# NethermindEth/latticefold

Hardware: AMD Instinct MI355X
Metric: folding-prover steps/sec (one NIFSProver::prove per step), GoldilocksRingNTT (higher is better)
Workload: dtype u64; 1 GPU; C4: GoldilocksRingNTT R1CS->CCS, m=N=2^20 rows, wit_len=262144, L=4, B=2^16, b=2, K=16, kappa=26, t=3; parallelism=replicas x1

## Files before the change

### latticefold_amd/csrc/lf_ctx.h

```cpp
#pragma once
#include <hip/hip_runtime.h>
#include <assert.h>
#include <string.h>

#include <atomic>
#include <chrono>
#include <condition_variable>
#include <functional>
#include <future>
#include <thread>
#include <map>
#include <memory>
#include <mutex>
#include <string>
#include <vector>

#include "../../include/lfhip.h"
#include "bb_capi.h"
#include "lf_ctx_core.h"
#include "lf_common.h"
#include "lf_dist.h"
#include "lf_kernels.h"
#include "lf_sb.h"
#include "lf_verify.h"
// ... 243 lines not shown
        if (tr) { tr->t.set_basis(nullptr, nullptr); if (tr->bb) tr->bb->set_basis(nullptr, nullptr); }
    }
    const u64 *ring_in(const u64 *p, size_t elems) {
        if (!p) return p;
        keep.emplace_back(new std::vector<u64>(p, p + elems * RE));
        c->xb.to_int(keep.back()->data(), elems * 8);
        return keep.back()->data();
    }
    const u64 *ext_in(const u64 *p, size_t n) {
        if (!p) return p;
        keep.emplace_back(new std::vector<u64>(p, p + n * TAU));
        c->xb.to_int(keep.back()->data(), n);
        return keep.back()->data();
    }
    void ring_out(u64 *p, size_t elems) { if (p) c->xb.to_ext(p, elems * 8); }
    void ext_out(u64 *p, size_t n) { if (p) c->xb.to_ext(p, n); }
    void transcript(lf_transcript *t) {
        tr = t;
        if (t->bb) t->bb->set_basis(c->xb.T, c->xb.Ti);
        else t->t.set_basis(c->xb.T, c->xb.Ti);
    }
};
#define LF_XB(c) ((c) && (c)->xb.on && !t_xb_active)
int fold_impl(lf_ctx *c, Transcript &tr, SideState *S , u64 *lcccs_out, lf_witness **w_out, u64 *proof);
int commit_download(lf_ctx *c, const u64 *dev, size_t words, u64 *host);
int commit_parts_i8g(lf_ctx *c, const unsigned char *D, size_t ldn, u32 NP, u64 *out_dev);
int sb_cut_parts(lf_ctx *c, const lf_witness *wit, const char *name, const unsigned char **D);
void fold_draw_rho(lf_ctx *c, Transcript &tr, const u64 *eta, std::vector<u64> &rho_c, std::vector<u64> &rho, std::vector<int8_t> &rho8);
void fold_instance_host(lf_ctx *c, const std::vector<Fq3> &pt, const u64 *theta, const u64 *eta, const std::vector<u64> &rho_c, const std::vector<u64> &rho, SideState *S,
                        u64 *lcccs_out);
int fold_impl_sb(lf_ctx *c, Transcript &tr, SideState *S , u64 *lcccs_out, lf_witness **w_out, u64 *proof);
int sb_fold_round_abi(lf_ctx *c, const u64 *t5, const u64 *F, size_t n, const Fq3Const *d_mu, u64 *evals_out);
int dot_batch_dev(lf_ctx *c, const u64 *X, size_t ldx, u32 na, const u64 *Y, size_t ldy, u32 nb, size_t n, u64 *dpart, u64 *od, hipStream_t st = nullptr,
                         const char *tag = "", unsigned char *yb_pre = nullptr);
int coef_eval_dev(lf_ctx *c, const int32_t *planes, size_t n, const u64 *eq, size_t ldeq, u32 K, int mode_bits, u64 *partial, u64 *od, size_t ldp,
                         const lf_witness *wit = nullptr);
int lin_tail_rounds(lf_ctx *c, Transcript &tr, const u64 *cur, const u64 *cure, size_t n, u64 *tout, u64 *partial, u32 round, Fq3 *point,
                           u64 *msgs, u32 deg, const std::function<void(u32)> *after_round);
int build_z(lf_ctx *c, const int32_t *planes, u32 K, int mode_bits, const u64 *heads, u64 *z, size_t w0 = 0, size_t wcnt = (size_t)-1,
            const unsigned char *D = nullptr );
bool lcccs_point(const lf_params &P, const u64 *lcccs, std::vector<Fq3> &pt);
#pragma GCC visibility pop
```

### latticefold_amd/csrc/lf_dot_i8.hip

```cpp
#include <hip/hip_runtime.h>
#include <cstdlib>
#include "lf_field.cuh"
#include "lf_kernels.h"

namespace lf {
static inline size_t dcdiv(size_t a, size_t b) { return (a + b - 1) / b; }
typedef int v4i __attribute__((ext_vector_type(4)));

__device__ __forceinline__ u32 dot_perm(u32 hi, u32 lo, u32 sel) {
#if defined(__HIP_DEVICE_COMPILE__)
    return __builtin_amdgcn_perm(hi, lo, sel);
#else
    return 0;
#endif
}
__device__ __forceinline__ u64 dot_digits(u64 w) {
    u64 s = w + 0x8080808080808080ull;
    if (s < w) s += 0xFFFFFFFFull;
    return s ^ 0x8080808080808080ull;
}

__global__ void __launch_bounds__(256) k_dot_pack_y(const u64 *Y, size_t ldy, u32 nb, size_t n, size_t lead, size_t ldq, unsigned char *YB) {
    __shared__ u64 sm[4][64];
    const u32 lane = threadIdx.x & 63, wave = threadIdx.x >> 6;
    constexpr u32 PER_WAVE = 8;
    const size_t blocks = ldq / 64, groups = (blocks + PER_WAVE - 1) / PER_WAVE, wid = (size_t)blockIdx.x * 4 + wave;
    if (wid >= (size_t)nb * 24 * groups) return;
    const u32 wp = (u32)(wid / groups);
    const u32 b = wp / 24, slot = (wp % 24) / 3, cq = wp % 3;
    const u64 *src_row = Y + ((size_t)b * 24 + 3 * slot + cq) * ldy;
    unsigned char *dst_rows = YB + ((size_t)slot * 72 + (b * 3 + cq) * 8) * ldq;
    const u32 v = lane >> 3, c0 = 8 * (lane & 7);
    const unsigned char *src = (const unsigned char *)&sm[wave][0];
    for (u32 k = 0; k < PER_WAVE; k++) {
        const size_t blk = (wid % groups) * PER_WAVE + k;
        if (blk >= blocks) break;
        const size_t i0 = blk * 64, i = i0 + lane;
        sm[wave][lane] = (i >= lead && i < n) ? dot_digits(src_row[i]) : 0;
        __builtin_amdgcn_fence(__ATOMIC_RELEASE, "wavefront");
        __builtin_amdgcn_wave_barrier();
        u64 o = 0;
#pragma unroll
        for (int t = 0; t < 8; t++) {
            const u32 pos = c0 + t, col = 8 * ((pos & 15) >> 1) + 2 * (pos >> 4) + (pos & 1);
            o |= (u64)src[col * 8 + v] << (8 * t);
        }
        *(u64 *)(dst_rows + (size_t)v * ldq + i0 + c0) = o;
        __builtin_amdgcn_fence(__ATOMIC_ACQUIRE, "wavefront");
        __builtin_amdgcn_wave_barrier();
    }
}

struct DotI8Args {
    const u64 *X;
    size_t ldx, n;
    u32 na;
    const unsigned char *YB;
    size_t ldq;
    u32 nrows_y;
    u32 nsteps, steps_per_chunk, chunks;
    int32_t *part;
};

__device__ __forceinline__ void dot_load_x(const u64 *xrow, size_t iw, u32 g, size_t n, bool xlive, u64 (&dst)[16]) {
    if (xlive && iw + 64 <= n) {
#pragma unroll
        for (int t = 0; t < 8; t++) {
            const ulonglong2 p = *(const ulonglong2 *)(xrow + iw + 8 * t + 2 * g);
            dst[2 * t] = p.x; dst[2 * t + 1] = p.y;
        }
    } else {
#pragma unroll
        for (int e = 0; e < 16; e++) {
            const size_t i = iw + 8 * (e >> 1) + 2 * g + (e & 1);
            dst[e] = (xlive && i < n) ? xrow[i] : 0;
        }
    }
}
__device__ __forceinline__ void dot_load_y(const unsigned char *yb, size_t ldq, size_t i0, u32 row, u32 nrows_y, v4i (&b)[5]) {
#pragma unroll
    for (int nt = 0; nt < 5; nt++) {
        const u32 r = 16 * nt + row;
        b[nt] = r < nrows_y ? *(const v4i *)(yb + (size_t)r * ldq + i0) : v4i{0, 0, 0, 0};
    }
}
__device__ __forceinline__ void dot_step(v4i (&acc)[8][5], const u64 (&raw)[16], const v4i (&b)[5]) {
    u64 w[16];
#pragma unroll
    for (int t = 0; t < 16; t++) w[t] = dot_digits(raw[t]);
    constexpr u32 SEL_LO = 0x0C0C0400u, SEL_PAIR = 0x05040100u;
#pragma unroll
    for (int u = 0; u < 8; u++) {
        u32 op[4];
#pragma unroll
        for (int j = 0; j < 4; j++) {
            const u32 ub = u & 3;
            const u32 h0 = u < 4 ? (u32)w[4 * j] : (u32)(w[4 * j] >> 32), h1 = u < 4 ? (u32)w[4 * j + 1] : (u32)(w[4 * j + 1] >> 32);
            const u32 h2 = u < 4 ? (u32)w[4 * j + 2] : (u32)(w[4 * j + 2] >> 32), h3 = u < 4 ? (u32)w[4 * j + 3] : (u32)(w[4 * j + 3] >> 32);
            const u32 sel = SEL_LO + ub * 0x0101u;
            const u32 p01 = dot_perm(h1, h0, sel), p23 = dot_perm(h3, h2, sel);
            op[j] = dot_perm(p23, p01, SEL_PAIR);
        }
        const v4i av = v4i{(int)op[0], (int)op[1], (int)op[2], (int)op[3]};
#pragma unroll
        for (int nt = 0; nt < 5; nt++) acc[u][nt] = __builtin_amdgcn_mfma_i32_16x16x64_i8(av, b[nt], acc[u][nt], 0, 0, 0);
    }
}
__global__ void __launch_bounds__(256) __attribute__((amdgpu_waves_per_eu(1, 1))) k_dot_i8(DotI8Args a) {
    const u32 lane = threadIdx.x & 63, wave = threadIdx.x >> 6, row = lane & 15, g = lane >> 4;
    const u32 L = blockIdx.x, combo = (L % 8) + 8 * (L / 24), cz = (L / 8) % 3;
    const u32 slot = combo % 8, unit = slot * 3 + cz;
    const u32 chunk = (combo / 8) * 4 + wave;
    v4i acc[8][5];
#pragma unroll
    for (int u = 0; u < 8; u++)
#pragma unroll
        for (int nt = 0; nt < 5; nt++) acc[u][nt] = v4i{0, 0, 0, 0};
    if (chunk >= a.chunks) return;
    const u32 s0 = chunk * a.steps_per_chunk, s1 = s0 + a.steps_per_chunk < a.nsteps ? s0 + a.steps_per_chunk : a.nsteps;
    const u64 *xrow = a.X + ((size_t)row * 24 + 3 * slot + cz) * a.ldx;
    const bool xlive = row < a.na;
    const unsigned char *yb = a.YB + (size_t)slot * 72 * a.ldq;
    const u32 last = s1 > s0 ? s1 - 1 : s0;
    auto colw = [&](u32 st) { return (size_t)(st < last ? st : last) * 64; };
    u64 xa[16], xn[16], xm[16];
    v4i ba[5], bn[5], bm[5];
    dot_load_x(xrow, colw(s0), g, a.n, xlive, xa); dot_load_y(yb, a.ldq, colw(s0) + 16 * g, row, a.nrows_y, ba);
    dot_load_x(xrow, colw(s0 + 1), g, a.n, xlive && s0 + 1 < s1, xn); dot_load_y(yb, a.ldq, colw(s0 + 1) + 16 * g, row, a.nrows_y, bn);
    auto ldx = [&](u32 st, u64 (&dst)[16]) { dot_load_x(xrow, colw(st), g, a.n, xlive && st < s1, dst); };
    for (u32 st = s0; st < s1; st += 3) {
        ldx(st + 2, xm); dot_load_y(yb, a.ldq, colw(st + 2) + 16 * g, row, a.nrows_y, bm);
        dot_step(acc, xa, ba);
        ldx(st + 3, xa); dot_load_y(yb, a.ldq, colw(st + 3) + 16 * g, row, a.nrows_y, ba);
        dot_step(acc, xn, bn);
        ldx(st + 4, xn); dot_load_y(yb, a.ldq, colw(st + 4) + 16 * g, row, a.nrows_y, bn);
        dot_step(acc, xm, bm);
    }
    int32_t *o = a.part + ((size_t)unit * a.chunks + chunk) * (8 * 5 * 256);
#pragma unroll
    for (int u = 0; u < 8; u++)
#pragma unroll
        for (int nt = 0; nt < 5; nt++) *(v4i *)(o + ((size_t)u * 5 + nt) * 256 + lane * 4) = acc[u][nt];
}

__global__ void __launch_bounds__(256) k_dot_i8_sum(const int32_t *part, u32 chunks, long long *tot) {
    const u32 e = blockIdx.x * 256 + threadIdx.x, unit = blockIdx.y;
    long long s = 0;
    for (u32 ch = 0; ch < chunks; ch++) s += part[((size_t)unit * chunks + ch) * 10240 + e];
    tot[(size_t)unit * 10240 + e] = s;
}

__global__ void __launch_bounds__(32) k_dot_i8_finish(const long long *tot, u32 na, u32 nb, u64 nu, u64 *out, u32 nb_out, u32 b0) {
    __shared__ u64 sm[24];
    const u32 o = blockIdx.x, t = threadIdx.x;
    const u32 comp = o % 3, slot = (o % 24) / 3, b = (o / 24) % nb, av = o / (24 * nb);
    if (t < 24) {
        const u32 cz = t >> 3, u = t & 7, cq = (comp + 3 - cz) % 3;
        const long long *tu = tot + (size_t)(slot * 3 + cz) * 10240;
        __int128 inner = 0;
#pragma unroll
        for (u32 v = 0; v < 8; v++) {
            const u32 col = (b * 3 + cq) * 8 + v, nt = col >> 4, cl = col & 15;
            inner += (__int128)tu[((size_t)u * 5 + nt) * 256 + (cl + 16 * (av >> 2)) * 4 + (av & 3)] << (8 * v);
        }
        u64 val = fq_from_s128((u64)inner, (int64_t)(inner >> 64));
        u64 pw = 1;
        for (u32 i = 0; i < u; i++) pw = fq_mul(pw, 256);
        val = fq_mul(val, pw);
        if (cz + cq >= 3) val = fq_mul(val, nu);
        sm[t] = val;
    }
    __syncthreads();
    if (t == 0) {
        u64 res = 0;
        for (int i = 0; i < 24; i++) res = fq_add(res, sm[i]);
        out[((size_t)av * nb_out + b0 + b) * 24 + 3 * slot + comp] = fq_canon(res);
    }
}

size_t dot_i8_yb_bytes(size_t n) { return (size_t)8 * 72 * (dcdiv(n, 64) * 64) + 64; }
static u32 dot_i8_chunks(size_t nsteps) {
    size_t want = 40;
    if (want > nsteps) want = nsteps;
    const size_t spc = dcdiv(nsteps, want);
    return (u32)dcdiv(nsteps, spc);
}
size_t dot_i8_part_words(size_t) { return (size_t)24 * 40 * 10240; }
size_t dot_i8_tot_words() { return (size_t)24 * 10240; }
int launch_dot_pack_y(const u64 *X, const u64 *Y, size_t ldy, u32 nb, size_t n, unsigned char *YB, hipStream_t s) {
    if (nb < 1 || nb > 3 || n < 64 || (((size_t)X) & 7)) return -1;
    const size_t lead = (((size_t)X) & 15) ? 1 : 0;
    Y -= lead; n += lead;
    const size_t ldq = dcdiv(n, 64) * 64;
    hipLaunchKernelGGL(k_dot_pack_y, dim3((unsigned)dcdiv((size_t)nb * 24 * dcdiv(ldq / 64, 8), 4)), dim3(256), 0, s, Y, ldy, nb, n, lead, ldq, YB);
    return 0;
}
int launch_dot_batch_i8(const DevCrt &t, const u64 *X, size_t ldx, u32 na, const u64 *Y, size_t ldy, u32 nb, size_t n, unsigned char *YB, int32_t *part,
                        long long *tot, u64 *out, hipStream_t s, bool y_packed, u32 nb_out, u32 b0) {
    if (!nb_out) nb_out = nb;
    if (na < 1 || na > 16 || nb < 1 || nb > 3 || n < 64 || (ldx & 1) || (((size_t)X) & 7)) return -1;
    const size_t lead = (((size_t)X) & 15) ? 1 : 0;
    X -= lead; Y -= lead; n += lead;
    const size_t ldq = dcdiv(n, 64) * 64;
    if (dcdiv(ldq / 64, dot_i8_chunks(ldq / 64)) >= 2048) return -1;
    if (!y_packed) hipLaunchKernelGGL(k_dot_pack_y, dim3((unsigned)dcdiv((size_t)nb * 24 * dcdiv(ldq / 64, 8), 4)), dim3(256), 0, s, Y, ldy, nb, n, lead, ldq, YB);
    DotI8Args a;
    a.X = X; a.ldx = ldx; a.n = n; a.na = na; a.YB = YB; a.ldq = ldq; a.nrows_y = 24 * nb;
    a.nsteps = (u32)(ldq / 64);
    a.chunks = dot_i8_chunks(a.nsteps);
    a.steps_per_chunk = (u32)dcdiv(a.nsteps, a.chunks);
    a.part = part;
    hipLaunchKernelGGL(k_dot_i8, dim3((unsigned)dcdiv(a.chunks, 4) * 24), dim3(256), 0, s, a);
    hipLaunchKernelGGL(k_dot_i8_sum, dim3(40, 24), dim3(256), 0, s, part, a.chunks, tot);
    hipLaunchKernelGGL(k_dot_i8_finish, dim3(na * nb * 24), dim3(32), 0, s, tot, na, nb, t.nu, out, nb_out, b0);
    return 0;
}
}
```

### latticefold_amd/csrc/lf_fold.cpp

```cpp
#include "lf_ring_host.h"

static int tail_host_rounds(lf_ctx *c, Transcript &tr, u32 epoch, u32 nr, u32 npts, bool dev_transcript, u64 *msgs, Fq3 *pt,
                            const std::function<void(u32)> *after_round = nullptr, u32 round0 = 0) {
    TailMail *mail = c->tail_mail;
    const auto t_start = std::chrono::steady_clock::now();
    double host_us = 0, wait_us = 0;
    auto t_mark = t_start;
    const bool tl_on = t_tl && t_tl->on;
    for (u32 i = 0; i < nr; i++) {
        u32 spins = 0;
        while (__atomic_load_n(&mail->msg_seq[i], __ATOMIC_ACQUIRE) != epoch) {
            __builtin_ia32_pause();
            if ((++spins & 0xfff) == 0) {
                if (__atomic_load_n(&mail->err, __ATOMIC_RELAXED) == epoch ||
                    std::chrono::duration<double>(std::chrono::steady_clock::now() - t_start).count() > 10.0) {
                    __atomic_store_n(&mail->abort_seq, epoch, __ATOMIC_RELEASE);
                    (void)hipStreamSynchronize(c->stream());
                    return LF_ERR_HIP;
                }
            }
        }
        if (tl_on) { auto nw = std::chrono::steady_clock::now(); wait_us += std::chrono::duration<double, std::micro>(nw - t_mark).count(); t_mark = nw; }
        u64 *evs = msgs + (size_t)i * npts * 24;
        memcpy(evs, (const void *)mail->msg[i], (size_t)npts * 24 * 8);
// ... 626 lines not shown
    {
        size_t c0, cnt;
        shard_slice(c, n, &c0, &cnt);
        if (s1f != c->stream() && P.t > 1) {
            HIPCHK(hipEventRecord(c->ev_prep[0], c->stream()));
            HIPCHK(hipStreamWaitEvent(s1f, c->ev_prep[0], 0));
        }
        for (u32 j = 0; j < P.t; j++)
            launch_spmv_t_eq(c->dcrt, c->d_colptr[j], c->d_rowidx[j], c->d_valT[j], eq0, m, q + (size_t)j * 24 * n, n, (j & 1) ? s1f : c->stream(), c0, cnt);
        if (s1f != c->stream() && P.t > 1) {
            HIPCHK(hipEventRecord(c->ev_prep[1], s1f));
            HIPCHK(hipStreamWaitEvent(c->stream(), c->ev_prep[1], 0));
        }
    }
    u64 *fsm;
    RET(c->tbuf("fold_small", (size_t)K2 * 72 + (size_t)K2 * P.t * 24 + 64, &fsm));
    RET(c->pin((size_t)K2 * 72 + (size_t)K2 * P.t * 24));
    u64 *hp = c->h_pin_ref();
    u64 *d_theta = fsm, *d_eta = fsm + (size_t)K2 * 72;
    if (P.s >= 4 && curF && ldF == 2 && !c->tn.theta_eval) launch_fix_final(c->dcrt, curF, K2 * 3 * 8, f3c(pt[P.s - 1]), d_theta, c->stream());
    else
    {
        size_t i0, cnt;
        shard_slice(c, N, &i0, &cnt);
        for (int sd = 0; sd < 2; sd++) RET(coef_eval_dev(c, S[sd].planes + i0, cnt, eq0 + i0, m, K, 1, red, d_theta + (size_t)sd * K * 72, N));
        RET(exchange_modsum_dev(c, d_theta, (size_t)K2 * 72));
    }
    HIPCHK(hipMemcpyAsync(hp, d_theta, (size_t)K2 * 72 * 8, hipMemcpyDeviceToHost, c->stream()));
    if (!c->ev_theta) HIPCHK(hipEventCreateWithFlags(&c->ev_theta, hipEventDisableTiming));
    HIPCHK(hipEventRecord(c->ev_theta, c->stream()));
    {
        size_t c0, cnt;
        shard_slice(c, n, &c0, &cnt);
        hipStream_t s1 = (t_lane == 0 && c->sh_world == 1 && c->st_lane[1]) ? c->st_lane[1] : c->stream();
        if (s1 != c->stream()) {
            if (!c->ev_prep[0]) { HIPCHK(hipEventCreateWithFlags(&c->ev_prep[0], hipEventDisableTiming)); HIPCHK(hipEventCreateWithFlags(&c->ev_prep[1], hipEventDisableTiming)); }
            unsigned char *ybq = nullptr;
            if (!c->tn.dot_valu && cnt >= c->tn.dot_min && P.t <= 3 && K <= 16 && ((((size_t)(S[0].z + c0)) ^ ((size_t)(S[1].z + c0))) & 15) == 0) {
                RET(c->tbuf("dot_yb", dot_i8_yb_bytes(n + 1), &ybq));
                if (launch_dot_pack_y(S[0].z + c0, q + c0, n, P.t, cnt, ybq, c->stream()) != 0) ybq = nullptr;
            }
            HIPCHK(hipEventRecord(c->ev_prep[0], c->stream()));
            HIPCHK(hipStreamWaitEvent(s1, c->ev_prep[0], 0));
            u64 *dpart1;
            RET(c->tbuf("dot_partial1", dot_partial_words(K, P.t), &dpart1));
            RET(dot_batch_dev(c, S[1].z + c0, n, K, q + c0, n, P.t, cnt, dpart1, d_eta + (size_t)K * P.t * 24, s1, "_1", ybq));
            HIPCHK(hipEventRecord(c->ev_prep[1], s1));
            RET(dot_batch_dev(c, S[0].z + c0, n, K, q + c0, n, P.t, cnt, dpart, d_eta, nullptr, "", ybq));
            HIPCHK(hipStreamWaitEvent(c->stream(), c->ev_prep[1], 0));
        } else
            for (int sd = 0; sd < 2; sd++) RET(dot_batch_dev(c, S[sd].z + c0, n, K, q + c0, n, P.t, cnt, dpart, d_eta + (size_t)sd * K * P.t * 24));
        RET(exchange_modsum_dev(c, d_eta, (size_t)K2 * P.t * 24));
    }
    HIPCHK(hipMemcpyAsync(hp + (size_t)K2 * 72, d_eta, (size_t)K2 * P.t * 24 * 8, hipMemcpyDeviceToHost, c->stream()));
    HIPCHK(hipEventSynchronize(c->ev_theta));
    memcpy(theta, hp, (size_t)K2 * 72 * 8);
    {
        HostTimer ht(c);
        tr.absorb_ring(theta, (size_t)K2 * 3);
    }
    HIPCHK(hipStreamSynchronize(c->stream()));
    memcpy(eta, hp + (size_t)K2 * 72, (size_t)K2 * P.t * 24 * 8);
    TL_MARK(" theta/eta");
    std::vector<u64> rho_c, rho;
    std::vector<int8_t> rho8;
    fold_draw_rho(c, tr, eta, rho_c, rho, rho8);
    int8_t *d_rho;
    RET(c->tbuf("c_rho", (size_t)K2 * 24 + 64, &d_rho));
    HIPCHK(hipMemcpyAsync(d_rho, rho8.data(), rho8.size(), hipMemcpyHostToDevice, c->stream()));
    int32_t *npl;
    RET(lf_planes_alloc(c, N * 24 * 4, &npl));
    LF_TRACE(c, "theta/eta");
    launch_fold_witness(S[0].planes, S[1].planes, N, K, d_rho, npl, c->stream());
    u64 *nf = nullptr, *nw = nullptr;
    const size_t nf_bytes = N * 24 * 8, nw_bytes = (size_t)P.wit_len * 24 * 8;
    RET(lf_planes_alloc(c, nf_bytes, (int32_t **)&nf));
    RET(lf_planes_alloc(c, nw_bytes, (int32_t **)&nw));
    launch_recompose_crt(c->dcrt, npl, N, (u32)N, 1, P.B, 1, 0, nf, N, 0, c->stream());
    launch_recompose_crt(c->dcrt, npl, N, P.wit_len, P.L, P.B, 1, 0, nw, P.wit_len, 0, c->stream());
    LF_TRACE(c, "fold_witness");
    TL_MARK("  eta absorbed, rho drawn, fold_witness enqueued");

    fold_instance_host(c, pt, theta, eta, rho_c, rho, S, lcccs_out);
    TL_MARK("  folded instance on the host");
// ... 82 lines not shown
```

### latticefold_amd/csrc/lf_fold_sb.cpp

```cpp
#include "lf_ring_host.h"


static void sb_compose_message(const u64 *norm, const u64 *g, u32 deg, u64 *evs) {
    for (u32 w = 0; w < 24; w++) {
        u64 g0 = g[w], g1 = g[24 + w], g2 = g[48 + w];
        evs[w] = fq_add(norm[w], g0);
        evs[24 + w] = fq_add(norm[24 + w], g1);
        evs[48 + w] = fq_add(norm[48 + w], g2);
        for (u32 X = 3; X <= deg; X++) {
            const u64 d = fq_sub(g2, g1), g3 = fq_add(fq_add(fq_add(d, d), d), g0);
            evs[(size_t)X * 24 + w] = fq_add(norm[(size_t)X * 24 + w], g3);
            g0 = g1; g1 = g2; g2 = g3;
        }
    }
}

int sb_fold_round_abi(lf_ctx *c, const u64 *t5, const u64 *F, size_t n, const Fq3Const *d_mu, u64 *evals_out) {
    const lf_params &P = c->P;
    const u32 deg = 2 * P.b;
    FoldRoundArgs a;
    a.eqL = t5; a.eqR = t5 + 3 * n; a.eqB = t5 + 6 * n; a.G1 = t5 + 9 * n; a.G2 = t5 + 33 * n;
    a.ld = n; a.n = n; a.p0 = 0; a.pcnt = n / 2; a.pF0 = 0;
    u64 *partial, *partial_g, *od;
    RET(c->tbuf("sb_round_partial", sb_round_partial_words(), &partial));
// ... 104 lines not shown
            a.ld = nn; a.n = nn; a.pcnt = nn / 2;
        }
        size_t ev = c->ev_begin(0);
        if (launch_sb_round(c->dcrt, P.b, a, curF, ldF, S[0].D, S[1].D, ldn, N, K, d_mu, partial, od, c->stream()) != 0) return LF_ERR_HIP;
        launch_fold_round_g(c->dcrt, a, partial_g, od + sb_round_out_words(), c->stream());
        if (hipGetLastError() != hipSuccess) return LF_ERR_HIP;
        c->ev_end(ev);
        RET(down_small(c, od, h.size(), h.data()));
        u64 *evs = msgs + (size_t)(round - 1) * (deg + 1) * 24;
        HostTimer ht(c);
        sb_compose_message(h.data(), h.data() + sb_round_out_words(), deg, evs);
        pt[round - 1] = sc_round_transcript(tr, evs, deg + 1);
    }
    c->ev_end(ph);

    ph = c->ev_begin(15);
    u64 *theta = proof + (size_t)P.s * (deg + 1) * 24, *eta = theta + (size_t)K2 * 72;
    u64 *eq0, *q, *dpart, *fsm;
    RET(c->tbuf("fold_eq0", 3 * m, &eq0));
    RET(c->tbuf("dec_q", (size_t)P.t * 24 * n, &q));
    RET(c->tbuf("dot_partial", dot_partial_words(K, P.t), &dpart));
    RET(c->tbuf("fold_small", (size_t)K2 * 72 + (size_t)K2 * P.t * 24 + 64, &fsm));
    RET(build_eq_dev(c, pt.data(), P.s, eq0));
    u64 *d_theta = fsm, *d_eta = fsm + (size_t)K2 * 72;
    if (curF && ldF == 2) launch_fix_final(c->dcrt, curF, K2 * 3 * 8, f3c(pt[P.s - 1]), d_theta, c->stream());
    else {
        u64 *sbp;
        RET(c->tbuf("sb_eval_partial", sb_eval_partial_words(K), &sbp));
        for (int sd = 0; sd < 2; sd++)
            if (launch_sb_eval(S[sd].D, ldn, N, eq0, m, K, sbp, d_theta + (size_t)sd * K * 72, c->stream()) != 0) return LF_ERR_HIP;
    }
    for (u32 j = 0; j < P.t; j++) launch_spmv_t_eq(c->dcrt, c->d_colptr[j], c->d_rowidx[j], c->d_valT[j], eq0, m, q + (size_t)j * 24 * n, n, c->stream());
    if (hipGetLastError() != hipSuccess) return LF_ERR_HIP;
    for (int sd = 0; sd < 2; sd++) RET(dot_batch_dev(c, S[sd].z, n, K, q, n, P.t, n, dpart, d_eta + (size_t)sd * K * P.t * 24));
    RET(down_small(c, fsm, (size_t)K2 * 72 + (size_t)K2 * P.t * 24, theta));
    {
        HostTimer ht(c);
        tr.absorb_ring(theta, (size_t)K2 * 3);
    }
    std::vector<u64> rho_c, rho;
    std::vector<int8_t> rho8;
    fold_draw_rho(c, tr, eta, rho_c, rho, rho8);
    int8_t *d_rho;
    RET(c->tbuf("c_rho", (size_t)K2 * 24 + 64, &d_rho));
    RET(c->h2d_small(d_rho, rho8.data(), rho8.size()));
    int32_t *npl;
    RET(lf_planes_alloc(c, N * 24 * 4, &npl));
    u64 *nf = nullptr, *nw = nullptr;
    const size_t nf_bytes = N * 24 * 8, nw_bytes = (size_t)P.wit_len * 24 * 8;
    RET(lf_planes_alloc(c, nf_bytes, (int32_t **)&nf));
    RET(lf_planes_alloc(c, nw_bytes, (int32_t **)&nw));
    if (launch_sb_fold_witness(S[0].D, S[1].D, ldn, N, K, d_rho, npl, c->stream()) != 0) return LF_ERR_HIP;
    launch_recompose_crt(c->dcrt, npl, N, (u32)N, 1, P.B, 1, 0, nf, N, 0, c->stream());
    launch_recompose_crt(c->dcrt, npl, N, P.wit_len, P.L, P.B, 1, 0, nw, P.wit_len, 0, c->stream());
    if (hipGetLastError() != hipSuccess) return LF_ERR_HIP;
    fold_instance_host(c, pt, theta, eta, rho_c, rho, S, lcccs_out);
    HIPCHK(hipStreamSynchronize(c->stream()));
    *w_out = new lf_witness{c, npl, N, c->device, N * 24 * 4};
    (*w_out)->f_ntt = nf; (*w_out)->f_bytes = nf_bytes; (*w_out)->w_ccs = nw; (*w_out)->w_bytes = nw_bytes;
    c->ev_end(ph);
    return LF_OK;
}
```

### latticefold_amd/csrc/lf_kernels.h

```cpp
#pragma once
#include "lf_ajtai_i8.h"
#include "lf_sv_rounds.h"
#include <hip/hip_runtime.h>

#include "lf_host.h"

namespace lf {

struct DevCrt {
    u64 nu;
    int nu2p40;
    u64 w4, w2, w10, w1, w7, w5, w11;
    int slot_of_pos[8], pos1[8], pos2[8];
    u64 tw1[8], tw2[8];
};
DevCrt make_dev_crt(const CrtTables &T);

struct Fq3Const { u64 c[3]; };

void launch_aos_to_soa(const u64 *aos, u64 *soa, size_t n, hipStream_t s);
void launch_soa_to_aos(const u64 *soa, u64 *aos, size_t n, hipStream_t s);
void launch_fill_uniform(u64 *dst, size_t words, u64 seed, size_t start, hipStream_t s);
void launch_fill_ajtai(u64 *A, u32 kappa, size_t n, size_t n_total, size_t col0, u64 seed, hipStream_t s, u32 row0 = 0);

// ... 14 lines not shown
void launch_recompose_crt(const DevCrt &t, const int32_t *planes, size_t n_planes, u32 wit_len, u32 L, u64 B, u32 K,
                          int mode_bits, u64 *out, size_t ldz, size_t off, hipStream_t s);
void launch_linf(const u64 *coef, size_t n, u64 *out_max, hipStream_t s);


void launch_build_eq(const DevCrt &t, const Fq3Const *r_dev , u32 nv, u64 *eq , hipStream_t s);
size_t build_eq_scratch_words(u32 nv);
void launch_build_eq2(const DevCrt &t, const Fq3Const *r_dev, u32 nv, u64 *scratch, u64 *eq, hipStream_t s);
void launch_spmv(const DevCrt &t, const u32 *rowptr, const u32 *col, const u64 *val , const u64 *z,
                 size_t ldz, u64 *out, size_t m, int accumulate, hipStream_t s, size_t r0 = 0, size_t rcnt = (size_t)-1 );
void launch_spmv_sum(const DevCrt &t, u32 nm, const u32 *const *rowptr, const u32 *const *col, const u64 *const *val, const u64 *z,
                     size_t z_stride, size_t ldz, u64 *out, size_t m, hipStream_t s, size_t r0 = 0, size_t rcnt = (size_t)-1 );
void launch_spmv_rows(const DevCrt &t, u32 nm, const u32 *const *rowptr, const u32 *const *col, const u64 *const *val, const u64 *z, size_t z_stride, size_t n,
                      u64 *zaos, u64 *out, size_t m, int accumulate, hipStream_t s, size_t r0 = 0, size_t rcnt = (size_t)-1);
void launch_spmv_t_eq(const DevCrt &t, const u32 *colptr, const u32 *rowidx, const u64 *val, const u64 *eq, size_t m,
                      u64 *q, size_t n, hipStream_t s, size_t c0 = 0, size_t ccnt = (size_t)-1 );
void launch_dot_batch(const DevCrt &t, const u64 *X, size_t ldx, u32 na, const u64 *Y, size_t ldy, u32 nb, size_t n,
                      u64 *partial, u64 *out, hipStream_t s);
size_t dot_partial_words(u32 na, u32 nb);
void launch_dot_eq(const DevCrt &t, const u64 *X, size_t ldx, u32 na, const u64 *eq, size_t ldeq, size_t n, u64 *partial,
                   u64 *out, hipStream_t s);
void launch_coef_eval(const DevCrt &t, const int32_t *planes, size_t n, const u64 *eq, size_t ldeq, u32 K, int mode_bits,
                      u64 *partial, u64 *out, hipStream_t s, size_t ldp = 0);
size_t coef_eval_partial_words(u32 K);
void launch_lincomb_z(const DevCrt &t, const u64 *z, size_t ldz, u32 K, const Fq3Const *coef_dev , u32 tt, size_t n,
                      u64 *out, hipStream_t s, u32 per_slot = 0);
void launch_add_fhat_comb(const DevCrt &t, const int32_t *planes, size_t n_planes, u32 K, const Fq3Const *apow_dev ,
                          u64 *G, size_t m, hipStream_t s, size_t r0 = 0, size_t rcnt = (size_t)-1 );

void launch_fix_ring(const DevCrt &t, const u64 *in, u64 *out, size_t n_in, Fq3Const r, hipStream_t s);
void launch_fix_fq3(const DevCrt &t, const u64 *in, u64 *out, size_t n_in, Fq3Const r, hipStream_t s);
size_t dot_i8_yb_bytes(size_t n);
size_t dot_i8_part_words(size_t n);
size_t dot_i8_tot_words();
int launch_dot_batch_i8(const DevCrt &t, const u64 *X, size_t ldx, u32 na, const u64 *Y, size_t ldy, u32 nb, size_t n, unsigned char *YB, int32_t *part,
                        long long *tot, u64 *out, hipStream_t s, bool y_packed = false, u32 nb_out = 0, u32 b0 = 0);
int launch_dot_pack_y(const u64 *X, const u64 *Y, size_t ldy, u32 nb, size_t n, unsigned char *YB, hipStream_t s);
void launch_vs_combine(const u64 *vs , u32 K, u64 *v , hipStream_t s);
void launch_fix_final(const DevCrt &t, const u64 *in , u32 rows3, Fq3Const r, u64 *out , hipStream_t s);

struct LinCombDesc {
    u32 t, q;
    u32 S_off[9];
    u32 S_idx[16];
    u64 c[8][24];
    int c_unit[8];
    u32 first[8];
    u32 ms[8];
};
void launch_lin_round(const DevCrt &t, const LinCombDesc &desc, const u64 *mz, size_t ld, const u64 *eq, size_t ldeq, size_t n,
                      u32 deg, u64 *partial, u64 *out, hipStream_t s, u32 max_blocks = 0, u32 split_xmask = 0 );
void launch_lin_round_fused(const DevCrt &t, const LinCombDesc &desc, const u64 *mz_prev, size_t ld_prev, const u64 *eq_prev, size_t ldeq_prev, Fq3Const r, u64 *mz_out,
                            size_t ld_out, u64 *eq_out, size_t ldeq_out, size_t n, u32 deg, u64 *partial, u64 *out, hipStream_t s, u32 max_blocks = 0,
                            u32 split_xmask = 0 );
struct LinFix;
void launch_lin_round_wide(const DevCrt &t, const LinCombDesc &desc, const u64 *mz, size_t ld, const u64 *eq, size_t ldeq, size_t n, u32 deg, u64 *partial, u64 *out,
                           hipStream_t s, u32 max_blocks, u32 split_xmask, const LinFix *fx);
void launch_eq_pairsum(const u64 *in, size_t ld_in, size_t n_out, u64 *out, size_t ld_out, hipStream_t s);
void launch_eq_expand(const DevCrt &t, const u64 *E, size_t lde, size_t pairs, Fq3Const w0, Fq3Const w1, u64 *out, size_t ldo, hipStream_t s);

struct FoldRoundArgs {
    const u64 *eqL, *eqR, *eqB;
    const u64 *G1, *G2;
    size_t ld;
    size_t n;
    size_t p0, pcnt;
    size_t pF0;
};
void launch_fold_round1(const DevCrt &t, const FoldRoundArgs &a, const int32_t *planesL, const int32_t *planesR, size_t n_planes,
// ... 88 lines not shown
```

### latticefold_amd/csrc/lf_prove.cpp

```cpp
#include "lf_ring_host.h"


void sc_prologue(Transcript &tr, u32 nv, u32 deg) {
    tr.absorb_u64_as_ring(nv);
    tr.absorb_u64_as_ring(deg);
}
Fq3 sc_round_transcript(Transcript &tr, const u64 *evals, u32 npts) {
    tr.absorb_ring(evals, npts);
    Fq3 r = tr.get_challenge();
    tr.absorb_fq3_as_ring(r);
    return r;
}

static int run_lin_sumcheck(lf_ctx *c, Transcript &tr, const u64 *mz, const u64 *eqb, u64 *msgs , Fq3 *point, u64 *u_dev = nullptr,
                            const std::function<void(u32)> *after_round = nullptr, const Fq3 *beta = nullptr) {
    const lf_params &P = c->P;
    u32 deg = P.d + 1;
    size_t m = c->m;
    u64 *fx[2], *fe[2], *partial, *od;
    RET(c->tbuf("lin_fix0", (size_t)P.t * 24 * (m / 2), &fx[0]));
    RET(c->tbuf("lin_fix1", (size_t)P.t * 24 * (m / 4 ? m / 4 : 1), &fx[1]));
    RET(c->tbuf("lin_efix0", 3 * (m / 2), &fe[0]));
    RET(c->tbuf("lin_efix1", 3 * (m / 4 ? m / 4 : 1), &fe[1]));
    RET(c->tbuf("round_partial", round_partial_words(), &partial));
// ... 392 lines not shown
    for (u32 i = 0; i < P.kappa; i++) HostRing::sub(cm + (size_t)i * 24, &acc[(size_t)i * 24], y_s + (size_t)i * 24);
    return LF_OK;
}

int coef_eval_dev(lf_ctx *c, const int32_t *planes, size_t n, const u64 *eq, size_t ldeq, u32 K, int mode_bits, u64 *partial, u64 *od, size_t ldp,
                         const lf_witness *wit) {
    if (wit && mode_bits && planes == wit->planes && n == c->N)
        for (int sd = 0; sd < 2; sd++)
            if (c->bits_wit[sd] == wit && c->bits_ptr[sd]) {
                unsigned char *EB;
                int32_t *part, *tot;
                RET(c->tbuf("vs_eb", sv_eb_bytes(n / 2), &EB));
                RET(c->tbuf("vs_part", sv_vs_part_words(n, K), &part));
                RET(c->tbuf("vs_tot", sv_vs_tot_words(K), &tot));
                if (c->stream() != c->st_lane[1]) HIPCHK(hipStreamWaitEvent(c->stream(), c->bits_ev[sd], 0));
                if (launch_sv_vs(c->bits_ptr[sd], n, eq, ldeq, K, EB, part, tot, od, c->stream()) == 0) return LF_OK;
                break;
            }
    if (n >= 64) {
        unsigned char *EB;
        int32_t *part;
        long long *sum;
        const u32 nwg = 512;
        RET(c->tbuf("ce_eb", coef_eval_i8_eb_bytes(n), &EB));
        RET(c->tbuf("ce_part", coef_eval_i8_part_words(nwg), &part));
        RET(c->tbuf("ce_sum", (size_t)24 * 2 * 256, &sum));
        if (launch_coef_eval_i8(planes, ldp ? ldp : n, n, eq, ldeq, K, mode_bits, c->P.B / 2, EB, nwg, part, sum, od, c->stream()) == 0) return LF_OK;
    }
    launch_coef_eval(c->dcrt, planes, n, eq, ldeq, K, mode_bits, partial, od, c->stream(), ldp);
    return LF_OK;
}

int dot_batch_dev(lf_ctx *c, const u64 *X, size_t ldx, u32 na, const u64 *Y, size_t ldy, u32 nb, size_t n, u64 *dpart, u64 *od, hipStream_t st,
                         const char *tag, unsigned char *yb_pre) {
    if (!st) st = c->stream();
    if (!c->tn.dot_valu && n >= c->tn.dot_min && nb <= 8) {
        unsigned char *yb;
        int32_t *part;
        long long *tot;
        if (yb_pre && nb <= 3) yb = yb_pre;
        else
        RET(c->tbuf(std::string("dot_yb") + tag, dot_i8_yb_bytes(n + 1), &yb));
        RET(c->tbuf(std::string("dot_i8_part") + tag, dot_i8_part_words(n + 1), &part));
        RET(c->tbuf(std::string("dot_i8_tot") + tag, dot_i8_tot_words(), &tot));
        bool ok = true;
        const u32 gsz = nb <= 3 ? nb : 2;
        for (u32 b0 = 0; b0 < nb && ok; b0 += gsz)
            for (u32 a0 = 0; a0 < na && ok; a0 += 16)
                ok = launch_dot_batch_i8(c->dcrt, X + (size_t)a0 * 24 * ldx, ldx, na - a0 < 16 ? na - a0 : 16, Y + (size_t)b0 * 24 * ldy, ldy, nb - b0 < gsz ? nb - b0 : gsz, n, yb, part, tot,
                                         od + (size_t)a0 * nb * 24, st, yb_pre != nullptr && nb <= 3, nb, b0) == 0;
        if (ok) return LF_OK;
    }
    if (nb > 4) {
        u64 *tmp;
        RET(c->tbuf(std::string("dot_wide_tmp") + tag, (size_t)na * 4 * 24, &tmp));
        for (u32 b0 = 0; b0 < nb; b0 += 4) {
            const u32 cb = nb - b0 < 4 ? nb - b0 : 4;
            launch_dot_batch(c->dcrt, X, ldx, na, Y + (size_t)b0 * 24 * ldy, ldy, cb, n, dpart, tmp, st);
            HIPCHK(hipMemcpy2DAsync(od + (size_t)b0 * 24, (size_t)nb * 24 * 8, tmp, (size_t)cb * 24 * 8, (size_t)cb * 24 * 8, na, hipMemcpyDeviceToDevice, st));
        }
        return LF_OK;
    }
    launch_dot_batch(c->dcrt, X, ldx, na, Y, ldy, nb, n, dpart, od, st);
    return LF_OK;
}
static int decompose_prepare_z(lf_ctx *c, const u64 *xh , const lf_witness *wit, const char *side, SideState &S, u64 *proof) {
    const lf_params &P = c->P;
    u32 K = P.K;
    u64 *x_s = proof + (size_t)K * P.t * 24 + (size_t)K * 72, *z;
    int rc = c->tbuf("z_" + std::string(side), (size_t)K * 24 * c->n, &z);
    if (rc == LF_OK) {
        compute_x_s(c, xh, x_s);
        size_t w0 = 0, wcnt = (size_t)-1;
        const size_t Gw = (size_t)c->sh_world, hl = P.l + 1;
        if (shard_keep(c, 1, c->m)) {
            size_t c0, ccnt, lo, hi;
            shard_slice(c, c->n, &c0, &ccnt);
            rc = shard_col_range(c, (size_t)c->sh_rank * (c->m / Gw), c->m / Gw, &lo, &hi);
            if (hi <= lo) { lo = c0; hi = c0 + ccnt; }
            if (c0 < lo) lo = c0;
            if (c0 + ccnt > hi) hi = c0 + ccnt;
            w0 = lo > hl ? lo - hl : 0;
            const size_t w1 = hi > hl ? hi - hl : 0;
            wcnt = w1 > w0 ? w1 - w0 : 0;
// ... 401 lines not shown
```

Baseline: 59.35 steps/s.

## Fuse both sides' i8 dot batches into one paired launch with merged finish reduction

Replaces the two per-side i8 MFMA dot launches (previously split across two streams with events) with a single paired kernel that handles both witness sides in one grid. The kernel is rewritten to one-wave blocks with a templated X/Y prefetch depth, and the separate sum and finish kernels are merged into one finish kernel that reduces chunk partials in shared memory. The aim is to cut launch count, cross-stream sync and the extra reduction pass. In exchange there are fewer chunks per side and a new grid decomposition whose occupancy is untested.

New measurement: 59.35 steps/s (median of 2 runs). No clear change (-0.0%).

```diff
diff --git a/latticefold_amd/csrc/lf_ctx.h b/latticefold_amd/csrc/lf_ctx.h
--- a/latticefold_amd/csrc/lf_ctx.h
+++ b/latticefold_amd/csrc/lf_ctx.h
@@ -299,7 +299,7 @@
 int fold_impl_sb(lf_ctx *c, Transcript &tr, SideState *S , u64 *lcccs_out, lf_witness **w_out, u64 *proof);
 int sb_fold_round_abi(lf_ctx *c, const u64 *t5, const u64 *F, size_t n, const Fq3Const *d_mu, u64 *evals_out);
 int dot_batch_dev(lf_ctx *c, const u64 *X, size_t ldx, u32 na, const u64 *Y, size_t ldy, u32 nb, size_t n, u64 *dpart, u64 *od, hipStream_t st = nullptr,
-                         const char *tag = "", unsigned char *yb_pre = nullptr);
+                         const char *tag = "", unsigned char *yb_pre = nullptr, const u64 *X1 = nullptr, u64 *od1 = nullptr);
 int coef_eval_dev(lf_ctx *c, const int32_t *planes, size_t n, const u64 *eq, size_t ldeq, u32 K, int mode_bits, u64 *partial, u64 *od, size_t ldp,
                          const lf_witness *wit = nullptr);
 int lin_tail_rounds(lf_ctx *c, Transcript &tr, const u64 *cur, const u64 *cure, size_t n, u64 *tout, u64 *partial, u32 round, Fq3 *point,
diff --git a/latticefold_amd/csrc/lf_dot_i8.hip b/latticefold_amd/csrc/lf_dot_i8.hip
--- a/latticefold_amd/csrc/lf_dot_i8.hip
+++ b/latticefold_amd/csrc/lf_dot_i8.hip
@@ -6,6 +6,10 @@
 namespace lf {
 static inline size_t dcdiv(size_t a, size_t b) { return (a + b - 1) / b; }
 typedef int v4i __attribute__((ext_vector_type(4)));
+#ifndef DOT_XD
+#define DOT_XD 4
+#define DOT_YD 2
+#endif
 
 __device__ __forceinline__ u32 dot_perm(u32 hi, u32 lo, u32 sel) {
 #if defined(__HIP_DEVICE_COMPILE__)
@@ -52,9 +56,10 @@
 }
 
 struct DotI8Args {
-    const u64 *X;
+    const u64 *X[2];
     size_t ldx, n;
     u32 na;
+    u32 nside;
     const unsigned char *YB;
     size_t ldq;
     u32 nrows_y;
@@ -106,113 +111,140 @@
         for (int nt = 0; nt < 5; nt++) acc[u][nt] = __builtin_amdgcn_mfma_i32_16x16x64_i8(av, b[nt], acc[u][nt], 0, 0, 0);
     }
 }
-__global__ void __launch_bounds__(256) __attribute__((amdgpu_waves_per_eu(1, 1))) k_dot_i8(DotI8Args a) {
-    const u32 lane = threadIdx.x & 63, wave = threadIdx.x >> 6, row = lane & 15, g = lane >> 4;
-    const u32 L = blockIdx.x, combo = (L % 8) + 8 * (L / 24), cz = (L / 8) % 3;
-    const u32 slot = combo % 8, unit = slot * 3 + cz;
-    const u32 chunk = (combo / 8) * 4 + wave;
+template <int XD, int YD>
+__global__ void __launch_bounds__(64) __attribute__((amdgpu_waves_per_eu(1, 1))) k_dot_i8(DotI8Args a) {
+    const u32 lane = threadIdx.x, row = lane & 15, g = lane >> 4;
+    const u32 L = blockIdx.x, slot = L % 8, i = L / 8, cz = i % 3, j = i / 3, side = j % a.nside, chunk = j / a.nside;
+    const u32 unit = slot * 3 + cz;
     v4i acc[8][5];
 #pragma unroll
     for (int u = 0; u < 8; u++)
 #pragma unroll
         for (int nt = 0; nt < 5; nt++) acc[u][nt] = v4i{0, 0, 0, 0};
-    if (chunk >= a.chunks) return;
     const u32 s0 = chunk * a.steps_per_chunk, s1 = s0 + a.steps_per_chunk < a.nsteps ? s0 + a.steps_per_chunk : a.nsteps;
-    const u64 *xrow = a.X + ((size_t)row * 24 + 3 * slot + cz) * a.ldx;
+    const u64 *xrow = a.X[side] + ((size_t)row * 24 + 3 * slot + cz) * a.ldx;
     const bool xlive = row < a.na;
     const unsigned char *yb = a.YB + (size_t)slot * 72 * a.ldq;
     const u32 last = s1 > s0 ? s1 - 1 : s0;
     auto colw = [&](u32 st) { return (size_t)(st < last ? st : last) * 64; };
-    u64 xa[16], xn[16], xm[16];
-    v4i ba[5], bn[5], bm[5];
-    dot_load_x(xrow, colw(s0), g, a.n, xlive, xa); dot_load_y(yb, a.ldq, colw(s0) + 16 * g, row, a.nrows_y, ba);
-    dot_load_x(xrow, colw(s0 + 1), g, a.n, xlive && s0 + 1 < s1, xn); dot_load_y(yb, a.ldq, colw(s0 + 1) + 16 * g, row, a.nrows_y, bn);
+    u64 xb[XD][16];
+    v4i bb[YD][5];
     auto ldx = [&](u32 st, u64 (&dst)[16]) { dot_load_x(xrow, colw(st), g, a.n, xlive && st < s1, dst); };
-    for (u32 st = s0; st < s1; st += 3) {
-        ldx(st + 2, xm); dot_load_y(yb, a.ldq, colw(st + 2) + 16 * g, row, a.nrows_y, bm);
-        dot_step(acc, xa, ba);
-        ldx(st + 3, xa); dot_load_y(yb, a.ldq, colw(st + 3) + 16 * g, row, a.nrows_y, ba);
-        dot_step(acc, xn, bn);
-        ldx(st + 4, xn); dot_load_y(yb, a.ldq, colw(st + 4) + 16 * g, row, a.nrows_y, bn);
-        dot_step(acc, xm, bm);
-    }
-    int32_t *o = a.part + ((size_t)unit * a.chunks + chunk) * (8 * 5 * 256);
+    auto ldy = [&](u32 st, v4i (&dst)[5]) { dot_load_y(yb, a.ldq, colw(st) + 16 * g, row, a.nrows_y, dst); };
+#pragma unroll
+    for (int k = 0; k < XD - 1; k++) ldx(s0 + k, xb[k]);
+#pragma unroll
+    for (int k = 0; k < YD - 1; k++) ldy(s0 + k, bb[k]);
+    constexpr int U = XD % YD == 0 ? XD : XD * YD;
+    for (u32 st = s0; st < s1; st += U) {
+#pragma unroll
+        for (int k = 0; k < U; k++) {
+            ldx(st + k + XD - 1, xb[(k + XD - 1) % XD]);
+            ldy(st + k + YD - 1, bb[(k + YD - 1) % YD]);
+            dot_step(acc, xb[k % XD], bb[k % YD]);
+        }
+    }
+    int32_t *o = a.part + (((size_t)side * 24 + unit) * a.chunks + chunk) * (8 * 5 * 256);
 #pragma unroll
     for (int u = 0; u < 8; u++)
 #pragma unroll
         for (int nt = 0; nt < 5; nt++) *(v4i *)(o + ((size_t)u * 5 + nt) * 256 + lane * 4) = acc[u][nt];
 }
 
-__global__ void __launch_bounds__(256) k_dot_i8_sum(const int32_t *part, u32 chunks, long long *tot) {
-    const u32 e = blockIdx.x * 256 + threadIdx.x, unit = blockIdx.y;
-    long long s = 0;
-    for (u32 ch = 0; ch < chunks; ch++) s += part[((size_t)unit * chunks + ch) * 10240 + e];
-    tot[(size_t)unit * 10240 + e] = s;
-}
-
-__global__ void __launch_bounds__(32) k_dot_i8_finish(const long long *tot, u32 na, u32 nb, u64 nu, u64 *out, u32 nb_out, u32 b0) {
-    __shared__ u64 sm[24];
-    const u32 o = blockIdx.x, t = threadIdx.x;
-    const u32 comp = o % 3, slot = (o % 24) / 3, b = (o / 24) % nb, av = o / (24 * nb);
-    if (t < 24) {
-        const u32 cz = t >> 3, u = t & 7, cq = (comp + 3 - cz) % 3;
-        const long long *tu = tot + (size_t)(slot * 3 + cz) * 10240;
+__global__ void __launch_bounds__(256) k_dot_i8_finish(const int32_t *part, u32 chunks, u32 na, u32 nb, u64 nu, u64 *out0, u64 *out1, u32 nb_out, u32 b0) {
+    __shared__ long long tot[3 * 40 * 16][4];
+    __shared__ u64 sm[36][24];
+    const u32 aq = blockIdx.x & 3, slot = (blockIdx.x >> 2) & 7, side = blockIdx.x >> 5, t = threadIdx.x;
+    if (4 * aq >= na) return;
+    for (u32 e = t; e < 3 * 40 * 16; e += 256) {
+        const u32 cl = e & 15, tile = (e >> 4) % 40, cz = e / 640;
+        const int32_t *p = part + ((size_t)side * 24 + slot * 3 + cz) * chunks * 10240 + (size_t)tile * 256 + (cl + 16 * aq) * 4;
+        long long s0 = 0, s1 = 0, s2 = 0, s3 = 0;
+        for (u32 ch = 0; ch < chunks; ch++) {
+            const v4i v = *(const v4i *)(p + (size_t)ch * 10240);
+            s0 += v.x; s1 += v.y; s2 += v.z; s3 += v.w;
+        }
+        tot[e][0] = s0; tot[e][1] = s1; tot[e][2] = s2; tot[e][3] = s3;
+    }
+    __syncthreads();
+    const u32 nout = 4 * nb * 3;
+    for (u32 w = t; w < nout * 24; w += 256) {
+        const u32 o = w / 24, k = w % 24, comp = o % 3, b = (o / 3) % nb, a4 = o / (3 * nb);
+        const u32 cz = k >> 3, u = k & 7, cq = (comp + 3 - cz) % 3;
         __int128 inner = 0;
 #pragma unroll
         for (u32 v = 0; v < 8; v++) {
             const u32 col = (b * 3 + cq) * 8 + v, nt = col >> 4, cl = col & 15;
-            inner += (__int128)tu[((size_t)u * 5 + nt) * 256 + (cl + 16 * (av >> 2)) * 4 + (av & 3)] << (8 * v);
+            inner += (__int128)tot[(cz * 40 + u * 5 + nt) * 16 + cl][a4] << (8 * v);
         }
         u64 val = fq_from_s128((u64)inner, (int64_t)(inner >> 64));
         u64 pw = 1;
-        for (u32 i = 0; i < u; i++) pw = fq_mul(pw, 256);
+        for (u32 q = 0; q < u; q++) pw = fq_mul(pw, 256);
         val = fq_mul(val, pw);
         if (cz + cq >= 3) val = fq_mul(val, nu);
-        sm[t] = val;
+        sm[o][k] = val;
     }
     __syncthreads();
-    if (t == 0) {
-        u64 res = 0;
-        for (int i = 0; i < 24; i++) res = fq_add(res, sm[i]);
-        out[((size_t)av * nb_out + b0 + b) * 24 + 3 * slot + comp] = fq_canon(res);
+    if (t < nout) {
+        const u32 comp = t % 3, b = (t / 3) % nb, av = 4 * aq + t / (3 * nb);
+        if (av < na) {
+            u64 res = 0;
+            for (int q = 0; q < 24; q++) res = fq_add(res, sm[t][q]);
+            (side ? out1 : out0)[((size_t)av * nb_out + b0 + b) * 24 + 3 * slot + comp] = fq_canon(res);
+        }
     }
 }
 
 size_t dot_i8_yb_bytes(size_t n) { return (size_t)8 * 72 * (dcdiv(n, 64) * 64) + 64; }
-static u32 dot_i8_chunks(size_t nsteps) {
-    size_t want = 40;
+constexpr size_t DOT_I8_WAVES = 42;
+static u32 dot_i8_chunks(size_t nsteps, u32 nside) {
+    size_t want = DOT_I8_WAVES / nside;
     if (want > nsteps) want = nsteps;
     const size_t spc = dcdiv(nsteps, want);
     return (u32)dcdiv(nsteps, spc);
 }
-size_t dot_i8_part_words(size_t) { return (size_t)24 * 40 * 10240; }
-size_t dot_i8_tot_words() { return (size_t)24 * 10240; }
+size_t dot_i8_part_words(size_t) { return (size_t)24 * DOT_I8_WAVES * 10240; }
 int launch_dot_pack_y(const u64 *X, const u64 *Y, size_t ldy, u32 nb, size_t n, unsigned char *YB, hipStream_t s) {
     if (nb < 1 || nb > 3 || n < 64 || (((size_t)X) & 7)) return -1;
     const size_t lead = (((size_t)X) & 15) ? 1 : 0;
     Y -= lead; n += lead;
     const size_t ldq = dcdiv(n, 64) * 64;
     hipLaunchKernelGGL(k_dot_pack_y, dim3((unsigned)dcdiv((size_t)nb * 24 * dcdiv(ldq / 64, 8), 4)), dim3(256), 0, s, Y, ldy, nb, n, lead, ldq, YB);
-    return 0;
-}
-int launch_dot_batch_i8(const DevCrt &t, const u64 *X, size_t ldx, u32 na, const u64 *Y, size_t ldy, u32 nb, size_t n, unsigned char *YB, int32_t *part,
-                        long long *tot, u64 *out, hipStream_t s, bool y_packed, u32 nb_out, u32 b0) {
+    return hipGetLastError() == hipSuccess ? 0 : -2;
+}
+static int dot_i8_run(const DevCrt &t, const u64 *X0, const u64 *X1, size_t ldx, u32 na, const u64 *Y, size_t ldy, u32 nb, size_t n, unsigned char *YB, int32_t *part,
+                      u64 *out0, u64 *out1, hipStream_t s, bool y_packed, u32 nb_out, u32 b0) {
     if (!nb_out) nb_out = nb;
-    if (na < 1 || na > 16 || nb < 1 || nb > 3 || n < 64 || (ldx & 1) || (((size_t)X) & 7)) return -1;
-    const size_t lead = (((size_t)X) & 15) ? 1 : 0;
-    X -= lead; Y -= lead; n += lead;
+    const u32 nside = X1 ? 2 : 1;
+    if (na < 1 || na > 16 || nb < 1 || nb > 3 || n < 64 || (ldx & 1) || (((size_t)X0) & 7)) return -1;
+    if (X1 && ((((size_t)X0) ^ ((size_t)X1)) & 15)) return -1;
+    const size_t lead = (((size_t)X0) & 15) ? 1 : 0;
+    X0 -= lead; Y -= lead; n += lead;
+    if (X1) X1 -= lead;
     const size_t ldq = dcdiv(n, 64) * 64;
-    if (dcdiv(ldq / 64, dot_i8_chunks(ldq / 64)) >= 2048) return -1;
-    if (!y_packed) hipLaunchKernelGGL(k_dot_pack_y, dim3((unsigned)dcdiv((size_t)nb * 24 * dcdiv(ldq / 64, 8), 4)), dim3(256), 0, s, Y, ldy, nb, n, lead, ldq, YB);
     DotI8Args a;
-    a.X = X; a.ldx = ldx; a.n = n; a.na = na; a.YB = YB; a.ldq = ldq; a.nrows_y = 24 * nb;
+    a.X[0] = X0; a.X[1] = X1 ? X1 : X0; a.ldx = ldx; a.n = n; a.na = na; a.nside = nside; a.YB = YB; a.ldq = ldq; a.nrows_y = 24 * nb;
     a.nsteps = (u32)(ldq / 64);
-    a.chunks = dot_i8_chunks(a.nsteps);
+    a.chunks = dot_i8_chunks(a.nsteps, nside);
     a.steps_per_chunk = (u32)dcdiv(a.nsteps, a.chunks);
     a.part = part;
-    hipLaunchKernelGGL(k_dot_i8, dim3((unsigned)dcdiv(a.chunks, 4) * 24), dim3(256), 0, s, a);
-    hipLaunchKernelGGL(k_dot_i8_sum, dim3(40, 24), dim3(256), 0, s, part, a.chunks, tot);
-    hipLaunchKernelGGL(k_dot_i8_finish, dim3(na * nb * 24), dim3(32), 0, s, tot, na, nb, t.nu, out, nb_out, b0);
-    return 0;
-}
-}
+    if (a.steps_per_chunk >= 2048) return -1;
+    if (!y_packed) {
+        hipLaunchKernelGGL(k_dot_pack_y, dim3((unsigned)dcdiv((size_t)nb * 24 * dcdiv(ldq / 64, 8), 4)), dim3(256), 0, s, Y, ldy, nb, n, lead, ldq, YB);
+        if (hipGetLastError() != hipSuccess) return -2;
+    }
+    hipLaunchKernelGGL((k_dot_i8<DOT_XD, DOT_YD>), dim3(24 * nside * a.chunks), dim3(64), 0, s, a);
+    if (hipGetLastError() != hipSuccess) return -2;
+    hipLaunchKernelGGL(k_dot_i8_finish, dim3(32 * nside), dim3(256), 0, s, part, a.chunks, na, nb, t.nu, out0, out1, nb_out, b0);
+    return hipGetLastError() == hipSuccess ? 0 : -2;
+}
+int launch_dot_batch_i8(const DevCrt &t, const u64 *X, size_t ldx, u32 na, const u64 *Y, size_t ldy, u32 nb, size_t n, unsigned char *YB, int32_t *part, u64 *out,
+                        hipStream_t s, bool y_packed, u32 nb_out, u32 b0) {
+    return dot_i8_run(t, X, nullptr, ldx, na, Y, ldy, nb, n, YB, part, out, nullptr, s, y_packed, nb_out, b0);
+}
+int launch_dot_pair_i8(const DevCrt &t, const u64 *X0, const u64 *X1, size_t ldx, u32 na, const u64 *Y, size_t ldy, u32 nb, size_t n, unsigned char *YB,
+                       int32_t *part, u64 *out0, u64 *out1, hipStream_t s, bool y_packed, u32 nb_out, u32 b0) {
+    if (!X1) return -1;
+    return dot_i8_run(t, X0, X1, ldx, na, Y, ldy, nb, n, YB, part, out0, out1, s, y_packed, nb_out, b0);
+}
+}
diff --git a/latticefold_amd/csrc/lf_fold.cpp b/latticefold_amd/csrc/lf_fold.cpp
--- a/latticefold_amd/csrc/lf_fold.cpp
+++ b/latticefold_amd/csrc/lf_fold.cpp
@@ -682,24 +682,7 @@
     {
         size_t c0, cnt;
         shard_slice(c, n, &c0, &cnt);
-        hipStream_t s1 = (t_lane == 0 && c->sh_world == 1 && c->st_lane[1]) ? c->st_lane[1] : c->stream();
-        if (s1 != c->stream()) {
-            if (!c->ev_prep[0]) { HIPCHK(hipEventCreateWithFlags(&c->ev_prep[0], hipEventDisableTiming)); HIPCHK(hipEventCreateWithFlags(&c->ev_prep[1], hipEventDisableTiming)); }
-            unsigned char *ybq = nullptr;
-            if (!c->tn.dot_valu && cnt >= c->tn.dot_min && P.t <= 3 && K <= 16 && ((((size_t)(S[0].z + c0)) ^ ((size_t)(S[1].z + c0))) & 15) == 0) {
-                RET(c->tbuf("dot_yb", dot_i8_yb_bytes(n + 1), &ybq));
-                if (launch_dot_pack_y(S[0].z + c0, q + c0, n, P.t, cnt, ybq, c->stream()) != 0) ybq = nullptr;
-            }
-            HIPCHK(hipEventRecord(c->ev_prep[0], c->stream()));
-            HIPCHK(hipStreamWaitEvent(s1, c->ev_prep[0], 0));
-            u64 *dpart1;
-            RET(c->tbuf("dot_partial1", dot_partial_words(K, P.t), &dpart1));
-            RET(dot_batch_dev(c, S[1].z + c0, n, K, q + c0, n, P.t, cnt, dpart1, d_eta + (size_t)K * P.t * 24, s1, "_1", ybq));
-            HIPCHK(hipEventRecord(c->ev_prep[1], s1));
-            RET(dot_batch_dev(c, S[0].z + c0, n, K, q + c0, n, P.t, cnt, dpart, d_eta, nullptr, "", ybq));
-            HIPCHK(hipStreamWaitEvent(c->stream(), c->ev_prep[1], 0));
-        } else
-            for (int sd = 0; sd < 2; sd++) RET(dot_batch_dev(c, S[sd].z + c0, n, K, q + c0, n, P.t, cnt, dpart, d_eta + (size_t)sd * K * P.t * 24));
+        RET(dot_batch_dev(c, S[0].z + c0, n, K, q + c0, n, P.t, cnt, dpart, d_eta, nullptr, "", nullptr, S[1].z + c0, d_eta + (size_t)K * P.t * 24));
         RET(exchange_modsum_dev(c, d_eta, (size_t)K2 * P.t * 24));
     }
     HIPCHK(hipMemcpyAsync(hp + (size_t)K2 * 72, d_eta, (size_t)K2 * P.t * 24 * 8, hipMemcpyDeviceToHost, c->stream()));
diff --git a/latticefold_amd/csrc/lf_fold_sb.cpp b/latticefold_amd/csrc/lf_fold_sb.cpp
--- a/latticefold_amd/csrc/lf_fold_sb.cpp
+++ b/latticefold_amd/csrc/lf_fold_sb.cpp
@@ -160,7 +160,7 @@
     }
     for (u32 j = 0; j < P.t; j++) launch_spmv_t_eq(c->dcrt, c->d_colptr[j], c->d_rowidx[j], c->d_valT[j], eq0, m, q + (size_t)j * 24 * n, n, c->stream());
     if (hipGetLastError() != hipSuccess) return LF_ERR_HIP;
-    for (int sd = 0; sd < 2; sd++) RET(dot_batch_dev(c, S[sd].z, n, K, q, n, P.t, n, dpart, d_eta + (size_t)sd * K * P.t * 24));
+    RET(dot_batch_dev(c, S[0].z, n, K, q, n, P.t, n, dpart, d_eta, nullptr, "", nullptr, S[1].z, d_eta + (size_t)K * P.t * 24));
     RET(down_small(c, fsm, (size_t)K2 * 72 + (size_t)K2 * P.t * 24, theta));
     {
         HostTimer ht(c);
diff --git a/latticefold_amd/csrc/lf_kernels.h b/latticefold_amd/csrc/lf_kernels.h
--- a/latticefold_amd/csrc/lf_kernels.h
+++ b/latticefold_amd/csrc/lf_kernels.h
@@ -70,9 +70,10 @@
 void launch_fix_fq3(const DevCrt &t, const u64 *in, u64 *out, size_t n_in, Fq3Const r, hipStream_t s);
 size_t dot_i8_yb_bytes(size_t n);
 size_t dot_i8_part_words(size_t n);
-size_t dot_i8_tot_words();
-int launch_dot_batch_i8(const DevCrt &t, const u64 *X, size_t ldx, u32 na, const u64 *Y, size_t ldy, u32 nb, size_t n, unsigned char *YB, int32_t *part,
-                        long long *tot, u64 *out, hipStream_t s, bool y_packed = false, u32 nb_out = 0, u32 b0 = 0);
+int launch_dot_batch_i8(const DevCrt &t, const u64 *X, size_t ldx, u32 na, const u64 *Y, size_t ldy, u32 nb, size_t n, unsigned char *YB, int32_t *part, u64 *out,
+                        hipStream_t s, bool y_packed = false, u32 nb_out = 0, u32 b0 = 0);
+int launch_dot_pair_i8(const DevCrt &t, const u64 *X0, const u64 *X1, size_t ldx, u32 na, const u64 *Y, size_t ldy, u32 nb, size_t n, unsigned char *YB, int32_t *part,
+                       u64 *out0, u64 *out1, hipStream_t s, bool y_packed = false, u32 nb_out = 0, u32 b0 = 0);
 int launch_dot_pack_y(const u64 *X, const u64 *Y, size_t ldy, u32 nb, size_t n, unsigned char *YB, hipStream_t s);
 void launch_vs_combine(const u64 *vs , u32 K, u64 *v , hipStream_t s);
 void launch_fix_final(const DevCrt &t, const u64 *in , u32 rows3, Fq3Const r, u64 *out , hipStream_t s);
diff --git a/latticefold_amd/csrc/lf_prove.cpp b/latticefold_amd/csrc/lf_prove.cpp
--- a/latticefold_amd/csrc/lf_prove.cpp
+++ b/latticefold_amd/csrc/lf_prove.cpp
@@ -448,24 +448,35 @@
 }
 
 int dot_batch_dev(lf_ctx *c, const u64 *X, size_t ldx, u32 na, const u64 *Y, size_t ldy, u32 nb, size_t n, u64 *dpart, u64 *od, hipStream_t st,
-                         const char *tag, unsigned char *yb_pre) {
+                         const char *tag, unsigned char *yb_pre, const u64 *X1, u64 *od1) {
     if (!st) st = c->stream();
+    if (X1 && (c->tn.dot_valu || n < c->tn.dot_min || nb > 8 || n < 64 || ((((size_t)X) ^ ((size_t)X1)) & 15))) {
+        RET(dot_batch_dev(c, X, ldx, na, Y, ldy, nb, n, dpart, od, st, tag, yb_pre));
+        return dot_batch_dev(c, X1, ldx, na, Y, ldy, nb, n, dpart, od1, st, tag, yb_pre);
+    }
     if (!c->tn.dot_valu && n >= c->tn.dot_min && nb <= 8) {
         unsigned char *yb;
         int32_t *part;
-        long long *tot;
         if (yb_pre && nb <= 3) yb = yb_pre;
         else
         RET(c->tbuf(std::string("dot_yb") + tag, dot_i8_yb_bytes(n + 1), &yb));
         RET(c->tbuf(std::string("dot_i8_part") + tag, dot_i8_part_words(n + 1), &part));
-        RET(c->tbuf(std::string("dot_i8_tot") + tag, dot_i8_tot_words(), &tot));
-        bool ok = true;
+        int rc = 0;
         const u32 gsz = nb <= 3 ? nb : 2;
-        for (u32 b0 = 0; b0 < nb && ok; b0 += gsz)
-            for (u32 a0 = 0; a0 < na && ok; a0 += 16)
-                ok = launch_dot_batch_i8(c->dcrt, X + (size_t)a0 * 24 * ldx, ldx, na - a0 < 16 ? na - a0 : 16, Y + (size_t)b0 * 24 * ldy, ldy, nb - b0 < gsz ? nb - b0 : gsz, n, yb, part, tot,
-                                         od + (size_t)a0 * nb * 24, st, yb_pre != nullptr && nb <= 3, nb, b0) == 0;
-        if (ok) return LF_OK;
+        for (u32 b0 = 0; b0 < nb && rc == 0; b0 += gsz)
+            for (u32 a0 = 0; a0 < na && rc == 0; a0 += 16) {
+                const u32 ca = na - a0 < 16 ? na - a0 : 16, cb = nb - b0 < gsz ? nb - b0 : gsz;
+                const bool packed = yb_pre != nullptr && nb <= 3;
+                if (X1) rc = launch_dot_pair_i8(c->dcrt, X + (size_t)a0 * 24 * ldx, X1 + (size_t)a0 * 24 * ldx, ldx, ca, Y + (size_t)b0 * 24 * ldy, ldy, cb, n, yb, part,
+                                                od + (size_t)a0 * nb * 24, od1 + (size_t)a0 * nb * 24, st, packed, nb, b0);
+                else rc = launch_dot_batch_i8(c->dcrt, X + (size_t)a0 * 24 * ldx, ldx, ca, Y + (size_t)b0 * 24 * ldy, ldy, cb, n, yb, part, od + (size_t)a0 * nb * 24, st, packed, nb, b0);
+            }
+        if (rc == 0) return LF_OK;
+        if (rc != -1) return LF_ERR_HIP;
+    }
+    if (X1) {
+        RET(dot_batch_dev(c, X, ldx, na, Y, ldy, nb, n, dpart, od, st, tag, yb_pre));
+        return dot_batch_dev(c, X1, ldx, na, Y, ldy, nb, n, dpart, od1, st, tag, yb_pre);
     }
     if (nb > 4) {
         u64 *tmp;
```
